# shahcompbio/MultiModalMuSig.jl

Hardware: AMD Instinct MI355X
Metric: E-step docs/sec (higher is better)
Workload: dtype f64; 1 GPU; LDA K=10 alpha=eta=0.1, 10000 docs x 96 SNV terms (BASELINE configs[1]), nnz(rank 0)=913480, one EM iteration per step; docs_rank0=10000, docs_total=10000, terms=96, topics=10, allreduce=none, comm_nranks=1, devices_visible=1

## Files before the change

multimodalmusig.jl_amd/csrc/lda.hip:

```cpp
#include <memory>
#include "dev_math.h"
#include "mmm_logtab.h"
#include "mmm_exptab.h"
#include "mmm_internal.h"

namespace {

constexpr int kWavesPerBlock = 4;
constexpr int kBlock = kWavesPerBlock * MMM_WAVE;
constexpr int kMaxWavesE = 12;

struct LdaDev {
    int D, V, K;
    const int64_t* doc_ptr;
    const int2* tc;
    double alpha, eta;
    const int2* ell;
    const int* dense;
    int Vp;
    const unsigned short* dense16;
};

struct LdaCtl {
    unsigned int ticket;
    int stop;
    int stop_iter;
    int t;
    int n_hist;
    int wait_timeout;
    int pad[2];
};

struct Ring { double* s[3]; };

template <bool RB, class T>
__device__ __forceinline__ T* rep(T* p, size_t n) { return RB ? p + (size_t)blockIdx.y * n : p; }

__device__ __forceinline__ void cell_store(unsigned long long* c, double v, unsigned int seq)
{
    const unsigned long long bits = (unsigned long long)__double_as_longlong(v), tag = (unsigned long long)seq << 32;
    __hip_atomic_store(c, (bits & 0xffffffffull) | tag, __ATOMIC_RELAXED, __HIP_MEMORY_SCOPE_AGENT);
    __hip_atomic_store(c + 1, (bits >> 32) | tag, __ATOMIC_RELAXED, __HIP_MEMORY_SCOPE_AGENT);
// ... 25 lines not shown
#pragma unroll
        for (int j = 0; j < MAXJ; ++j) {
            if (pending & (1u << j)) {
                w0[j] = __hip_atomic_load(c + 2 * (lane + 64 * j), __ATOMIC_RELAXED, __HIP_MEMORY_SCOPE_AGENT);
                w1[j] = __hip_atomic_load(c + 2 * (lane + 64 * j) + 1, __ATOMIC_RELAXED, __HIP_MEMORY_SCOPE_AGENT);
            }
        }
#pragma unroll
        for (int j = 0; j < MAXJ; ++j) {
            if ((pending & (1u << j)) && (unsigned int)(w0[j] >> 32) == seq && (unsigned int)(w1[j] >> 32) == seq) {
                val[j] = __longlong_as_double((long long)((w0[j] & 0xffffffffull) | (w1[j] << 32)));
                pending &= ~(1u << j);
            }
        }
        if (pending) __builtin_amdgcn_s_sleep(1);
    }
    if (pending) ctl->wait_timeout = 1;
    double v = 0.0;
#pragma unroll
    for (int j = 0; j < MAXJ; ++j) v += val[j];
    return v;
}

constexpr int kIldaMaxI = 8, kIldaMaxSJ = 512;

struct EstepArgs {
    LdaDev c;
    const LdaCtl* ctl;
    Ring gamma, Elntheta, expElnbeta, beta;
    double* partial;
    double* llpart;
    int do_ll;
    int t;
    int pstride;
    const double* aexp;
};

#ifdef MMM_DIAG_STAMPS
__device__ unsigned long long g_lda_stamps[16];
#define MMM_STAMP(i)                                                                                         \
    do {                                                                                                     \
        unsigned long long t_;                                                                               \
        __builtin_amdgcn_sched_barrier(0);                                                                   \
        asm volatile("s_memtime %0\n\ts_waitcnt lgkmcnt(0)" : "=s"(t_)::"memory");                          \
        __builtin_amdgcn_sched_barrier(0);                                                                   \
        if (blockIdx.x == 0 && threadIdx.x == 0) g_lda_stamps[i] = t_;                                       \
        if ((i) == 0 || (i) == 7) {                                                                          \
            unsigned long long r_ = __builtin_amdgcn_s_memrealtime();                                        \
            if (blockIdx.x == 0 && threadIdx.x == 0) g_lda_stamps[8 + ((i) != 0)] = r_;                     \
            if (blockIdx.x == gridDim.x - 1 && threadIdx.x == 0) g_lda_stamps[10 + ((i) != 0)] = r_;        \
        }                                                                                                    \
    } while (0)
__device__ unsigned long long g_red_stamps[32];
__device__ unsigned long long g_ll_times[2][512];
#define MMM_LLSTAMP(which, lb)                                                                               \
    do {                                                                                                     \
        __builtin_amdgcn_sched_barrier(0);                                                                   \
        unsigned long long r_ = __builtin_amdgcn_s_memrealtime();                                            \
// ... 57 lines not shown
    bool theta_valid = false;
    bool attr_e[2] = {false, false}, attr_m = false, attr_mm[3] = {false, false, false};
    int cap_mm[3] = {-1, -1, -1}, cap_m = -1;
    DevBuf<unsigned long long> cells;
    DevBuf<unsigned long long> fcells;
    unsigned int kseq = 0;
    bool stop_seen = false;
    bool lag_ll = true;
    bool phi_table_beta = false;
    bool single_step = false;
    bool wide = false;
    DevBuf<int64_t> term_ptr;
    DevBuf<int2> tpost;
    DevBuf<double> aexp;
    DevBuf<double> aexp_next;
    int aexp_for = -1;
    bool pro_used = false;
    DevBuf<double> tabT;
    int stats_waves = 1;
    bool attr_big = false, attr_bigs = false;
    int grid_e = 1, waves_e = 8, grid_s = 1;
    size_t lds_e = 0, lds_tab = 0;
    bool block_stats = false;
    size_t lds_b = 0; bool attr_b = false;
    bool ilda = false;
    IldaDesc ids{};
    DevBuf<int> features;
    DevBuf<double> ilam[3], iEln[3], ibeta[3];
    int R = 1, sel = 0;
    std::vector<int> rep_t, rep_hist;
    PinnedCtl pin;
    LdaDev dev() const { return LdaDev{D, V, K, doc_ptr.p, tc.p, alpha, eta, tc_ell.p, (drows && !cnt16.p) ? cnt_dense.p : nullptr, 16 * SLs, cnt16.p}; }
    int cur() const { return t % 3; }
    Ring ring(DevBuf<double>* b) const { return Ring{{b[0].p, b[1].p, b[2].p}}; }
    double* tab(DevBuf<double>* b, int s) const { return b[s].p + (size_t)sel * V * K; }
    double* doc(DevBuf<double>* b, int s) const { return b[s].p + (size_t)sel * K * D; }
    LdaCtl* ctlp() const { return ctl.p + sel; }
    double* hist() const { return ll_hist.p + (size_t)sel * cap_hist; }
    size_t lds_red() const { return sizeof(double) * ((size_t)KP * V + 64 * (size_t)KP + MMM_LOGTAB_N); }
    int docs_per_ll_block() const { return 16 * (MMM_WAVE / (KP <= 15 ? 16 : (KP <= 31 ? 32 : 64))); }
    void passes_enqueued(bool lag, bool table_beta)
    {
        inflight = true; lag_ll = lag; phi_table_beta = table_beta;
        if (!lag) ll_pending = false;
        phi_valid = false; phi_from_prev = true; gnext_valid = true; theta_valid = false;
    }
};

namespace {

int pick_kp(int K)
{
    static const int opts[] = {2, 4, 6, 8, 10, 12, 16, 20, 24, 32};
    for (int o : opts) if (K <= o) return o;
    if (K <= 64 * kLdaSlots) return (K + 1) & ~1;
// ... 27 lines not shown
{
    mmm_ctx* ctx = m->ctx;
    int nb = 0;
    MMM_HIP(ctx, hipOccupancyMaxActiveBlocksPerMultiprocessor(&nb, (const void*)kern, 1024, lds));
    *cap = nb * std::max(1, ctx->num_cu - 4);
    if (m->tune.resident_cap > 0) *cap = std::min(*cap, m->tune.resident_cap);
    return MMM_OK;
}

template <int KPV, int LV, bool LLV, int VT, bool SG, bool RB>
int go_estep3(mmm_lda* m, const EstepArgs& a)
{
    mmm_ctx* ctx = m->ctx;
    auto k = k_lda_estep<KPV, LV, LLV, VT, SG, RB>;
    if (!m->attr_e[LLV]) { int rc = set_lds(ctx, k, m->lds_e); if (rc) return rc; m->attr_e[LLV] = true; }
    hipLaunchKernelGGL(k, dim3(m->grid_e, RB ? m->R : 1), dim3(m->waves_e * MMM_WAVE), m->lds_e, ctx->stream, a);
    return MMM_OK;
}

template <int KPV, int VT, bool RB>
int go_estep_block(mmm_lda* m, const EstepArgs& a)
{
    mmm_ctx* ctx = m->ctx;
    auto k = k_lda_estep_block<KPV, VT, RB>;
    if (!m->attr_b) { int rc = set_lds(ctx, k, m->lds_b); if (rc) return rc; m->attr_b = true; }
    hipLaunchKernelGGL(k, dim3(m->grid_e, RB ? m->R : 1), dim3(m->waves_e * MMM_WAVE), m->lds_b, ctx->stream, a);
    return MMM_OK;
}

template <int KPV, int LV, bool LLV, int VT, bool RB>
int go_estep2(mmm_lda* m, const EstepArgs& a)
{
    if constexpr (LV == 16 && KPV <= 12 && !LLV) { if (m->single_step && m->block_stats) return go_estep_block<KPV, VT, RB>(m, a); }
    if constexpr (LV == 16 && KPV <= 12) { if (m->single_step) return go_estep3<KPV, LV, LLV, VT, true, RB>(m, a); }
    return go_estep3<KPV, LV, LLV, VT, false, RB>(m, a);
}

template <int KPV, int LV, bool LLV, bool RB = false>
int go_estep(mmm_lda* m, const EstepArgs& a)
{
    if constexpr (LV == 16 && (KPV == 8 || KPV == 10)) { if (m->V == 96) return go_estep2<KPV, LV, LLV, 96, RB>(m, a); }
    return go_estep2<KPV, LV, LLV, 0, RB>(m, a);
}

template <int KPV, int SLV, bool RB = false>
int go_dense(mmm_lda* m, const EstepArgs& a)
{
    if constexpr (KPV * SLV <= 64) {
        mmm_ctx* ctx = m->ctx;
        const bool c16 = m->cnt16.p != nullptr;
        auto k = c16 ? k_lda_estep_dense<KPV, SLV, true, RB> : k_lda_estep_dense<KPV, SLV, false, RB>;
        if (!m->attr_d) { int rc = set_lds(ctx, k, m->lds_d); if (rc) return rc; m->attr_d = true; }
        hipLaunchKernelGGL(k, dim3(m->grid_e, RB ? m->R : 1), dim3(m->waves_e * MMM_WAVE), m->lds_d, ctx->stream, a, (const int*)m->cnt_dense.p, (const unsigned short*)m->cnt16.p);
        return MMM_OK;
    } else return mmm_fail(m->ctx, MMM_ERR_UNSUPPORTED, "LDA: no dense-row build for KP=%d SL=%d", KPV, SLV);
}

int dense_slots(int V) { return V <= 32 ? 2 : (V <= 48 ? 3 : (V <= 96 ? 6 : (V <= 128 ? 8 : 0))); }

template <bool RB = false>
int launch_estep(mmm_lda* m, const EstepArgs& a)
{
    mmm_ctx* ctx = m->ctx;
    int rc = MMM_OK;
    if (m->dense && !a.do_ll) {
        MMM_KP_SWITCH(m, {
            if constexpr (KPV >= 4 && KPV <= 16) {
                switch (m->SL) {
                    case 2: rc = go_dense<KPV, 2, RB>(m, a); break;
                    case 3: rc = go_dense<KPV, 3, RB>(m, a); break;
                    case 6: rc = go_dense<KPV, 6, RB>(m, a); break;
                    default: rc = go_dense<KPV, 8, RB>(m, a); break;
                }
            }
        })
        if (rc) return rc;
        MMM_LAUNCH_CHECK(ctx);
        return MMM_OK;
    }
    if constexpr (RB) {
        if (m->wide || a.do_ll) return mmm_fail(ctx, MMM_ERR_UNSUPPORTED, "LDA batch: no batched build of the wide path / the E-step ll");
        MMM_KP_SWITCH(m, {
            if (m->L == 16) { if constexpr (KPV <= 16) rc = go_estep<KPV, 16, false, true>(m, a); }
            else if (m->L == 32) { if constexpr (KPV >= 16) rc = go_estep<KPV, 32, false, true>(m, a); }
            else { if constexpr (KPV == 32) rc = go_estep<KPV, 64, false, true>(m, a); }
        })
        if (rc) return rc;
// ... 1242 lines not shown
```

multimodalmusig.jl_amd/csrc/lda_estep.cuh:

```cuda
__device__ __forceinline__ void lds_wave_sync()
{
    __builtin_amdgcn_fence(__ATOMIC_SEQ_CST, "wavefront");
    __builtin_amdgcn_wave_barrier();
}

template <bool RB = false>
struct EstepPass {
    const double* __restrict__ gam; const double* __restrict__ gprev; double* __restrict__ gnext; double* __restrict__ Eln;
    const double* __restrict__ eB; const double* __restrict__ bprev;
    __device__ __forceinline__ explicit EstepPass(const EstepArgs& a)
        : gam(a.gamma.s[a.t % 3]), gprev(a.gamma.s[(a.t + 2) % 3]), gnext(a.gamma.s[(a.t + 1) % 3]), Eln(a.Elntheta.s[a.t % 3]),
          eB(a.expElnbeta.s[(a.t + 2) % 3]), bprev(a.beta.s[(a.t + 2) % 3])
    {
        if constexpr (RB) {
            const size_t KD = (size_t)a.c.K * a.c.D, VK = (size_t)a.c.V * a.c.K;
            gam = rep<RB>(gam, KD); gprev = rep<RB>(gprev, KD); gnext = rep<RB>(gnext, KD); Eln = rep<RB>(Eln, KD);
            eB = rep<RB>(eB, VK); bprev = rep<RB>(bprev, VK);
        }
    }
    static __device__ __forceinline__ int stop(const EstepArgs& a) { return rep<RB>(a.ctl, 1)->stop; }
    static __device__ __forceinline__ double* partial(const EstepArgs& a, const int K)
    {
        double* out = a.partial + (size_t)blockIdx.x * K * a.pstride;
        if constexpr (RB) out += (size_t)blockIdx.y * gridDim.x * K * a.pstride;
        return out;
    }
};

template <int KP, bool LL>
__device__ __forceinline__ void lda_chunk(const int2 tcv, const bool act, const int V, const double (&av)[KP], double (&acc)[KP],
                                          const double* __restrict__ sB, const double* __restrict__ sBeta,
                                          const double* __restrict__ myT, double* __restrict__ slab, double& ll_acc)
{
    const double n = (double)tcv.y;
    if (LL) {
        const double* bc = sBeta + tcv.x;
        double p0 = 0.0, p1 = 0.0;
#pragma unroll
        for (int k = 0; k + 1 < KP; k += 2) { p0 = fma(myT[k], bc[k * V], p0); p1 = fma(myT[k + 1], bc[(k + 1) * V], p1); }
        if (KP & 1) p0 = fma(myT[KP - 1], bc[(KP - 1) * V], p0);
        ll_acc = fma(n, dev_log_pos(p0 + p1), ll_acc);
        __builtin_amdgcn_sched_barrier(0);
    }
// ... 16 lines not shown
    double b[KP], s0 = 0.0, s1 = 0.0;
#pragma unroll
    for (int k = 0; k < KP; ++k) b[k] = av[k] * bcol[k * V];
#pragma unroll
    for (int k = 0; k + 1 < KP; k += 2) { s0 += b[k]; s1 += b[k + 1]; }
    if (KP & 1) s0 += b[KP - 1];
    const double r = act ? n * dev_rcp(s0 + s1) : 0.0;
#pragma unroll
    for (int k = 0; k < KP; ++k) { b[k] *= r; acc[k] += b[k]; }
    if (act) {
        double* scol = slab + tcv.x;
#pragma unroll
        for (int k = 0; k < KP; ++k) unsafeAtomicAdd(&scol[k * V], b[k]);
    }
}

template <int KP, int L, bool LL, int VT, bool SINGLE, bool RB = false>
__global__ __launch_bounds__(SINGLE ? kMaxWavesE * MMM_WAVE : 512, SINGLE ? 3 : 2) void k_lda_estep(EstepArgs a)
{
    extern __shared__ __attribute__((aligned(16))) double smem[];
    constexpr int G = MMM_WAVE / L;
    constexpr int PRE = (96 + L - 1) / L;
    MMM_STAMP(0);
    const int stop = EstepPass<RB>::stop(a);
    const EstepPass<RB> io(a);
    const int K = a.c.K, D = a.c.D;
    const int V = VT ? VT : a.c.V;
    const int NW = blockDim.x >> 6;
    const int tid = threadIdx.x, lane = tid & 63, wid = tid >> 6;
    const int g = lane / L, l = lane % L;
    double* sB = smem;
    double* sBeta = sB + (size_t)KP * V;
    double* sSlab = sBeta + (size_t)KP * V;
    double* sA = sSlab + (size_t)NW * KP * V;
    double* sT = sA + (size_t)NW * G * KP;
    double* slab = sSlab + (size_t)wid * KP * V;
    double* myA = sA + ((size_t)wid * G + g) * KP;
    double* myT = sT + ((size_t)wid * G + g) * KP;
    const int stride = gridDim.x * NW * G;
    int base = (blockIdx.x * NW + wid) * G;
    double ll_acc = 0.0;

    int d = base + g;
    bool valid = d < D;
    const bool ext = SINGLE && !LL && !RB && a.aexp != nullptr;
    double gk = ext ? ((valid && l < K) ? a.aexp[(size_t)d * K + l] : 0.0) : ((valid && l < K) ? io.gam[(size_t)d * K + l] : (l < K ? 1.0 : 0.0));
    double gp = (LL && valid && l < K) ? io.gprev[(size_t)d * K + l] : (l < K ? 1.0 : 0.0);
// ... 13 lines not shown
        if (LL) sBeta[i] = (i < K * V) ? io.bprev[i] : 0.0;
    }
    MMM_STAMP(1);

    int d1 = 0; bool valid1 = false; int64_t start1 = 0; int W1 = 0;
    if (!SINGLE) {
        d1 = base + stride + g; valid1 = (base + stride < D) && d1 < D;
        start1 = (valid1 && !rows) ? a.c.doc_ptr[d1] : 0;
        W1 = (valid1 && !rows) ? (int)(a.c.doc_ptr[d1 + 1] - start1) : 0;
    }
    int2 tcp[PRE];
    bool first = true;
    for (;;) {
        const int NCHR = VT ? (VT + L - 1) / L : (V + L - 1) / L;
        const int nch = rows ? NCHR : (W + L - 1) / L;
        const int rot = nch > 0 ? g % nch : 0;
        const int2* __restrict__ tcd = a.c.tc + start;
        int nchmax = nch;
        if (!rows) {
            if (G >= 2) nchmax = max(nchmax, __shfl_xor(nchmax, 32, MMM_WAVE));
            if (G >= 4) nchmax = max(nchmax, __shfl_xor(nchmax, 16, MMM_WAVE));
            nchmax = __builtin_amdgcn_readfirstlane(nchmax);
        }
        if (SINGLE || first) lda_row_read<L, PRE, true, true, true>(a.c, drows, rows, d, valid, l, V, nch, rot, start, W, [&](int j, int w, int n) { tcp[j] = make_int2(w, n); });
        double el = 0.0;
        if (ext) { if (l < KP) myA[l] = gk; }
        else {
            el = lda_elntheta<L>(gk, g, l, K);
            if (l < KP) myA[l] = (l < K) ? ar_exp(el) : 0.0;
        }
        if (LL) {
            const double Sp = group_sum<L>(gp);
            if (l < KP) myT[l] = (l < K) ? gp / Sp : 0.0;
        }
        if (first) {
            if (stop) return;
            if (SINGLE) {
#pragma unroll
                for (int q = 0; q < TB; ++q) { const int i = tid + q * (int)blockDim.x; if (i < KP * V) sB[i] = tb[q]; }
                for (int i = tid + TB * (int)blockDim.x; i < KP * V; i += blockDim.x) sB[i] = (i < K * V) ? io.eB[i] : 0.0;
            }
            __syncthreads();
            first = false;
            MMM_STAMP(2);
        } else lds_wave_sync();
        if (!ext && valid && l < K) io.Eln[(size_t)d * K + l] = el;
        MMM_STAMP(3);
        int2 tcn[PRE];
        double gkn = 0.0, gpn = 0.0;
        int d2 = 0; bool valid2 = false; int64_t start2 = 0; int W2 = 0;
        const bool more = !SINGLE && base + stride < D;
        if (more) {
            const int nch1 = rows ? NCHR : (W1 + L - 1) / L;
            const int rot1 = nch1 > 0 ? g % nch1 : 0;
            lda_row_read<L, PRE, true, true, true>(a.c, drows, rows, d1, valid1, l, V, nch1, rot1, start1, W1, [&](int j, int w, int n) { tcn[j] = make_int2(w, n); });
            gkn = (valid1 && l < K) ? io.gam[(size_t)d1 * K + l] : (l < K ? 1.0 : 0.0);
            gpn = (LL && valid1 && l < K) ? io.gprev[(size_t)d1 * K + l] : (l < K ? 1.0 : 0.0);
            d2 = base + 2 * stride + g; valid2 = (base + 2 * stride < D) && d2 < D;
            start2 = (valid2 && !rows) ? a.c.doc_ptr[d2] : 0;
            W2 = (valid2 && !rows) ? (int)(a.c.doc_ptr[d2 + 1] - start2) : 0;
        }
        {
            double av[KP], acc[KP];
#pragma unroll
            for (int k = 0; k < KP; ++k) { av[k] = myA[k]; acc[k] = 0.0; }
            if (rows) {
#pragma unroll
                for (int j = 0; j < PRE; ++j) {
                    if (j < NCHR) {
                        int2 tcv = tcp[j];
                        const bool act = tcv.x >= 0;
                        tcv.x = act ? tcv.x : 0;
                        lda_chunk<KP, LL>(tcv, act, V, av, acc, sB, sBeta, myT, slab, ll_acc);
                    }
                }
            } else
#pragma unroll 2
            for (int j = 0; j < nchmax; ++j) {
// ... 49 lines not shown
        }
    }
    MMM_STAMP(7);
}


template <int KP>
__device__ __forceinline__ double lda_chunk_r(const int v, const double n, const bool act, const int V, const double (&av)[KP], double (&acc)[KP],
                                              const double* __restrict__ sB)
{
    const double* bcol = sB + v;
    double b[KP], s0 = 0.0, s1 = 0.0;
#pragma unroll
    for (int k = 0; k < KP; ++k) b[k] = bcol[k * V];
#pragma unroll
    for (int k = 0; k + 1 < KP; k += 2) { s0 = fma(av[k], b[k], s0); s1 = fma(av[k + 1], b[k + 1], s1); }
    if (KP & 1) s0 = fma(av[KP - 1], b[KP - 1], s0);
    const double r = act ? n * dev_rcp(s0 + s1) : 0.0;
#pragma unroll
    for (int k = 0; k < KP; ++k) acc[k] = fma(b[k], r, acc[k]);
    return r;
}

template <int KP, int VT, bool RB = false>
__global__ __launch_bounds__(kMaxWavesE * MMM_WAVE, 3) void k_lda_estep_block(EstepArgs a)
{
    static_assert(KP <= 12 && KP % 2 == 0, "topic pairs, table of <= 5 registers per thread");
    extern __shared__ __attribute__((aligned(16))) double smem[];
    constexpr int L = 16, G = MMM_WAVE / L, PRE = 96 / L;
    MMM_STAMP(0);
    const int stop = EstepPass<RB>::stop(a);
    const EstepPass<RB> io(a);
    const int K = a.c.K, D = a.c.D;
    const int V = VT ? VT : a.c.V;
    const int NCHR = VT ? (VT + L - 1) / L : (V + L - 1) / L;
    const int Vs = NCHR * L;
    const int NW = blockDim.x >> 6, ND = NW * G;
    const int tid = threadIdx.x, lane = tid & 63, wid = tid >> 6;
    const int g = lane / L, l = lane % L;
    double* sB = smem;
    double* sR = sB + (size_t)KP * V;
    double* sA = sR + (size_t)ND * Vs;
    double* myR = sR + (size_t)(wid * G + g) * Vs;
    double* myA = sA + (size_t)(wid * G + g) * KP;

    const int d = (blockIdx.x * NW + wid) * G + g;
    const bool valid = d < D;
    const bool ext = !RB && a.aexp != nullptr;
    const double gk = ext ? ((valid && l < K) ? a.aexp[(size_t)d * K + l] : 0.0) : ((valid && l < K) ? io.gam[(size_t)d * K + l] : (l < K ? 1.0 : 0.0));
    const bool drows = a.c.dense != nullptr || a.c.dense16 != nullptr;
    const bool rows = drows || a.c.ell != nullptr;
    const int64_t start = (valid && !rows) ? a.c.doc_ptr[d] : 0;
    const int W = (valid && !rows) ? (int)(a.c.doc_ptr[d + 1] - start) : 0;
    constexpr int TB = KP <= 10 ? 4 : 5;
    double tb[TB];
#pragma unroll
    for (int q = 0; q < TB; ++q) { const int i = tid + q * (int)blockDim.x; tb[q] = (i < K * V) ? io.eB[i] : 0.0; }
    if (!drows) for (int i = tid; i < ND * Vs; i += blockDim.x) sR[i] = 0.0;
    MMM_STAMP(1);

    int tv[PRE]; double tn[PRE];
    const int nch = rows ? NCHR : (W + L - 1) / L;
    lda_row_read<L, PRE, false, true, true>(a.c, drows, rows, d, valid, l, V, nch, 0, start, W, [&](int j, int w, int n) { tv[j] = w; tn[j] = (double)n; });
    double el = 0.0, al = gk;
    if (!ext) {
        el = lda_elntheta<L>(gk, g, l, K);
        al = (l < K) ? ar_exp(el) : 0.0;
    }
    if (l < KP) myA[l] = al;
    if (stop) return;
#pragma unroll
    for (int q = 0; q < TB; ++q) { const int i = tid + q * (int)blockDim.x; if (i < KP * V) sB[i] = tb[q]; }
    for (int i = tid + TB * (int)blockDim.x; i < KP * V; i += blockDim.x) sB[i] = (i < K * V) ? io.eB[i] : 0.0;
    __syncthreads();
    MMM_STAMP(2);
    if (!ext && valid && l < K) io.Eln[(size_t)d * K + l] = el;
    MMM_STAMP(3);
    double av[KP], acc[KP];
#pragma unroll
    for (int k = 0; k < KP; ++k) { av[k] = myA[k]; acc[k] = 0.0; }
    int nchmax = nch;
    if (!rows) {
        nchmax = max(nchmax, __shfl_xor(nchmax, 32, MMM_WAVE));
        nchmax = max(nchmax, __shfl_xor(nchmax, 16, MMM_WAVE));
        nchmax = __builtin_amdgcn_readfirstlane(nchmax);
    }
#pragma unroll
    for (int j = 0; j < PRE; ++j) {
        if (j < nchmax) {
            const bool act = tv[j] >= 0;
            const double r = lda_chunk_r<KP>(act ? tv[j] : 0, tn[j], act, V, av, acc, sB);
            if (drows) myR[j * L + l] = r;
            else if (act) myR[tv[j]] = r;
        }
    }
// ... 194 lines not shown
```

multimodalmusig.jl_amd/csrc/lda_reduce.cuh:

```cuda
struct ReduceArgs {
    const double* partial; const double* llpart; int nslab; int VK;
    double* stats;
    LdaCtl* ctl;
    int t;
    int hist_stride;
    double Nglobal, tol;
    double* ll_hist;
    int do_ll, conv_base, run_tail;
    int p2p; unsigned int p2p_seq; P2PArgs px;
    const double* llpart2; int n_ll, ll_in_k2;
    unsigned long long* ll_cells; unsigned int ll_seq;
};

template <bool RB>
__device__ __forceinline__ void rep_reduce(ReduceArgs& r)
{
    if constexpr (RB) {
        const size_t y = blockIdx.y;
        r.partial += y * r.nslab * r.VK; r.llpart += y * r.nslab; r.stats += y * (r.VK + 16);
        r.ctl += y; r.ll_hist += y * r.hist_stride; r.llpart2 += y * 512;
    }
}

__device__ void lda_pass_tail(const ReduceArgs& r)
// ... 12 lines not shown
    if (!stop) r.ctl->t = r.t;
    r.ctl->ticket = 0;
}

template <bool P2P>
__device__ __forceinline__ void lda_tail_block(const ReduceArgs& r, int lane)
{
    double v = 0.0;
    const bool from_parts = r.ll_in_k2 && !r.ll_cells;
    if (from_parts && r.do_ll) {
        for (int i = lane; i < r.n_ll; i += 64) v += r.llpart2[i];
        v = wave_sum(v);
    }
    if (lane != 0) return;
    if (from_parts) {
        if (r.do_ll) {
            if (P2P && r.p2p) { p2p_send(r.px, r.p2p_seq, r.VK, v); v = p2p_recv_sum(r.px, r.p2p_seq, r.VK, v); }
            r.stats[r.VK] = v;
        }
    } else if (P2P && r.p2p) r.stats[r.VK] = p2p_recv_sum(r.px, r.p2p_seq, r.VK, r.stats[r.VK]);
    lda_pass_tail(r);
}

template <int KP, int L>
__device__ void lda_ll_block(const LdaDev& c, const double* __restrict__ gprev, const double* __restrict__ bprev, double* llpart2, int lb, int nlb,
                             double* smem, unsigned long long* cell = nullptr, unsigned int seq = 0)
{
    __shared__ double s_w[16];
    const int tid = threadIdx.y * 16 + threadIdx.x, lane = tid & 63, wid = tid >> 6;
    constexpr int G = MMM_WAVE / L;
    const int g = lane / L, l = lane % L;
    const int K = c.K, V = c.V, D = c.D;
    double* sBeta = smem;
    double* myT = smem + (size_t)KP * V + ((size_t)wid * G + g) * KP;
    double* sLog = smem + (size_t)KP * V + (size_t)64 * KP;
    const int wslot = ((int64_t)nlb * 16 * G >= (int64_t)D) ? wid * nlb + lb : lb * 16 + wid, nslots = nlb * 16;
    int base = wslot * G;
    int d = base + g;
    bool valid = d < D;
    double gp = (valid && l < K) ? gprev[(size_t)d * K + l] : (l < K ? 1.0 : 0.0);
    constexpr int PRE = 128 / L;
    const bool dense = L == 16 && (c.dense != nullptr || c.dense16 != nullptr);
    const bool h16 = c.dense16 != nullptr;
    const bool ell = dense || c.ell != nullptr;
    int2 pre[PRE];
    const bool fast = L == 16 && dense && h16 && (int64_t)D * K * 8 < ((int64_t)1 << 32) && (int64_t)D * c.Vp * 2 < ((int64_t)1 << 32);
    unsigned wq[4] = {0u, 0u, 0u, 0u};
    const int lk = l < K ? l : K - 1;
    unsigned dl = valid ? (unsigned)d : 0u;
    if (fast) {
        const unsigned* row = at_byte((const unsigned*)c.dense16, (dl * 16u + (unsigned)l) * (unsigned)(c.Vp >> 4) * 2u);
#pragma unroll
        for (int j = 0; j < 4; ++j) wq[j] = row[j];
    } else if (ell) lda_row_read<L, PRE, false, false, false>(c, dense, ell, d, valid, l, V, 0, 0, 0, 0, [&](int j, int w, int n) { pre[j] = make_int2(w, n); });
    int64_t start = (!ell && valid) ? c.doc_ptr[d] : 0;
    int W = (!ell && valid) ? (int)(c.doc_ptr[d + 1] - start) : 0;
    for (int i = tid; i < KP * V; i += 1024) { const int v = i / KP, k = i - v * KP; sBeta[i] = (k < K) ? bprev[(size_t)k * V + v] : 0.0; }
    if (tid < MMM_LOGTAB_N) sLog[tid] = g_mmm_logtab[tid];
    MMM_RSTAMP(lb == 0 && tid == 0, 20);
    __syncthreads();
    MMM_RSTAMP(lb == 0 && tid == 0, 21);
    double acc = 0.0;
    if (fast) {
        const int nch = (V + L - 1) / L;
        const int stride = nslots * G;
        const unsigned slp2 = (unsigned)(c.Vp >> 4) * 2u;
        unsigned w[4];
#pragma unroll
        for (int j = 0; j < 4; ++j) w[j] = valid ? wq[j] : 0u;
        for (; base < D; base += stride) {
            const int dn = d + stride;
            const bool validn = base + stride < D && dn < D;
            const unsigned dnl = validn ? (unsigned)dn : dl;
            const double Sp = group_sum<L>(gp);
            lds_wave_sync();
            if (l < KP) myT[l] = (l < K) ? dev_div(gp, Sp) : 0.0;
            lds_wave_sync();
            double tv[KP];
#pragma unroll
            for (int k = 0; k < KP; ++k) tv[k] = myT[k];
            double gpn = *at_byte(gprev, (dnl * (unsigned)K + (unsigned)lk) * 8u);
            {
                const unsigned* row = at_byte((const unsigned*)c.dense16, (dnl * 16u + (unsigned)l) * slp2);
// ... 3 lines not shown
#pragma unroll
            for (int j = 0; j < 8; ++j) {
                if (j < nch) {
                    const unsigned cq = (j & 1) ? w[j / 2] >> 16 : w[j / 2] & 0xffffu;
                    const bool act = valid && j * L + l < V;
                    acc = lda_ll_term<KP>(tv, sBeta + (size_t)(act ? j * L + l : 0) * KP, act, (double)cq, sLog, acc);
                }
            }
            asm volatile("" : "+v"(acc) :: "memory");
            asm volatile("" : "+v"(gpn) :: "memory");
#pragma unroll
            for (int j = 0; j < 4; ++j) asm volatile("" : "+v"(wq[j]) :: "memory");
            d = dn; valid = validn; dl = dnl;
            gp = (valid && l < K) ? gpn : (l < K ? 1.0 : 0.0);
#pragma unroll
            for (int j = 0; j < 4; ++j) w[j] = valid ? wq[j] : 0u;
        }
    } else if (ell) {
        const int nch = (V + L - 1) / L;
        for (; base < D; base += nslots * G) {
            if (base != wslot * G) {
                d = base + g; valid = d < D;
                gp = (valid && l < K) ? gprev[(size_t)d * K + l] : (l < K ? 1.0 : 0.0);
                lda_row_read<L, PRE, false, false, false>(c, dense, ell, d, valid, l, V, 0, 0, 0, 0, [&](int j, int w, int n) { pre[j] = make_int2(w, n); });
            }
            const double Sp = group_sum<L>(gp);
            lds_wave_sync();
            if (l < KP) myT[l] = (l < K) ? dev_div(gp, Sp) : 0.0;
            lds_wave_sync();
            double tv[KP];
#pragma unroll
            for (int k = 0; k < KP; ++k) tv[k] = myT[k];
#pragma unroll
            for (int j = 0; j < PRE; ++j) {
                if (j >= nch) break;
                const int2 t = pre[j];
                const bool act = t.x >= 0;
                acc = lda_ll_term<KP>(tv, sBeta + (size_t)(act ? t.x : 0) * KP, act, (double)t.y, sLog, acc);
            }
        }
    } else
    for (; base < D; base += nslots * G) {
        if (base != wslot * G) {
            d = base + g; valid = d < D;
            gp = (valid && l < K) ? gprev[(size_t)d * K + l] : (l < K ? 1.0 : 0.0);
            start = valid ? c.doc_ptr[d] : 0;
            W = valid ? (int)(c.doc_ptr[d + 1] - start) : 0;
// ... 8 lines not shown
        for (int k = 0; k < KP; ++k) tv[k] = myT[k];
        int nchmax = (W + L - 1) / L;
        if (G >= 2) nchmax = max(nchmax, __shfl_xor(nchmax, 32, MMM_WAVE));
        if (G >= 4) nchmax = max(nchmax, __shfl_xor(nchmax, 16, MMM_WAVE));
        nchmax = __builtin_amdgcn_readfirstlane(nchmax);
        for (int j = 0; j < nchmax; ++j) {
            const int w = j * L + l;
            const bool act = w < W;
            const int2 t = act ? tcd[w] : make_int2(0, 0);
            acc = lda_ll_term<KP>(tv, sBeta + (size_t)t.x * KP, act, (double)t.y, sLog, acc);
        }
    }
    MMM_RSTAMP(lb == 0 && tid == 0, 22);
    acc = wave_sum(acc);
    if (lane == 0) s_w[wid] = acc;
    __syncthreads();
    MMM_RSTAMP(lb == 0 && tid == 0, 23);
    if (tid == 0) {
        double v = 0.0;
#pragma unroll
        for (int w = 0; w < 16; ++w) v += s_w[w];
        if (cell) cell_store(cell, v, seq); else llpart2[lb] = v;
    }
}

__device__ void lda_reduce_block(const ReduceArgs& r)
{
    __shared__ double sm[64][17];
    const int stop = r.ctl->stop;
    const int tx = threadIdx.x, ty = threadIdx.y;
    const int e = blockIdx.x * 16 + tx;
    double acc = 0.0;
    if (e < r.VK) for (int sl = ty; sl < r.nslab; sl += 64) acc += r.partial[(size_t)sl * r.VK + e];
    if (stop) {
        if (r.p2p && blockIdx.x == 0 && tx == 0 && ty == 0) p2p_send(r.px, r.p2p_seq, 0, 0.0);
        return;
    }
    sm[ty][tx] = acc;
    __syncthreads();
    if (ty < 8) {
        double v = 0.0;
#pragma unroll
        for (int j = 0; j < 8; ++j) v += sm[ty * 8 + j][tx];
        sm[ty * 8][tx] = v;
    }
    __syncthreads();
    if (ty == 0 && e < r.VK) {
        double v = 0.0;
#pragma unroll
        for (int j = 0; j < 8; ++j) v += sm[j * 8][tx];
        r.stats[e] = v;
        if (r.p2p) p2p_send(r.px, r.p2p_seq, e, v);
    }
    if (blockIdx.x == 0 && ty >= 4 && ty < 8 && r.ll_cells && r.do_ll) {
        const int lane = (ty * 16 + tx) & 63;
        double v = 0.0;
        v = cells_wait_sum(r.ll_cells, r.n_ll, lane, r.ll_seq, r.ctl);
// ... 41 lines not shown
    IldaDesc ds;
    double* ilam; double* iEln; double* ibeta;
    unsigned long long* fcells;
};

struct MergeArgs {
    int V; double eta;
    Ring lambda, Elnbeta, expElnbeta, beta;
    unsigned long long* cells;
    unsigned int seq;
    int nred;
    int ll_join;
    int n_ll;
    int epb, nredp;
    int pro;
    const double* pro_gamma; double* pro_Eln; double* pro_a;
};

template <int KP, bool P2P, bool ILDA>
__global__ __launch_bounds__(1024) void k_lda_reduce_ll_mstep(ReduceArgs r, LdaDev c, const double* gprev, const double* bprev, MergeArgs ms, IldaMerge im)
{
    extern __shared__ __attribute__((aligned(16))) double smem[];
    __shared__ double sm2[2][64][17];
    const int stop = r.ctl->stop;
    const int tx = threadIdx.x, ty = threadIdx.y, tid = ty * 16 + tx;
    MMM_RSTAMP(blockIdx.x == 1 && tid == 0, 0);
    MMM_RSTAMP(blockIdx.x == 0 && tid == 64, 8);
    MMM_RSTAMP((int)blockIdx.x == ms.nredp && tid == 0, 16);
    if ((int)blockIdx.x >= ms.nredp) {
        if (stop) return;
        constexpr int L = KP <= 15 ? 16 : (KP <= 31 ? 32 : 64);
        const int lb = (int)blockIdx.x - ms.nredp, n_ll = ms.n_ll;
        MMM_LLSTAMP(0, lb);
        double gnx = 0.0;
        int pd = 0;
        if constexpr (KP <= 12) {
            if (ms.pro) {
                const int lane = tid & 63, l = lane & 15;
                pd = ((tid >> 6) * n_ll + lb) * 4 + (lane >> 4);
                gnx = (pd < c.D && l < c.K) ? ms.pro_gamma[(size_t)pd * c.K + l] : (l < c.K ? 1.0 : 0.0);
            }
        }
        lda_ll_block<KP, L>(c, gprev, bprev, nullptr, lb, n_ll + (ms.ll_join ? ms.nredp - 1 : 0), smem, ms.cells + 2 * (ms.nred + lb), ms.seq);
        MMM_RSTAMP((int)blockIdx.x == ms.nredp && tid == 0, 17);
        MMM_LLSTAMP(1, lb);
        if constexpr (KP <= 12) {
            if (ms.pro) {
                const int lane = tid & 63, g = lane >> 4, l = lane & 15, K = c.K;
                const double el = lda_elntheta<16>(gnx, g, l, K);
                if (pd < c.D && l < K) { ms.pro_Eln[(size_t)pd * K + l] = el; ms.pro_a[(size_t)pd * K + l] = ar_exp(el); }
            }
        }
        return;
    }
    const int rbp = (int)blockIdx.x, epb = ms.epb;
    const int rb = rbp * epb + (ty < epb ? ty : 0);
    const int e = rb * 16 + tx;
    double acc = 0.0, acc1 = 0.0;
    {
        const int e0 = rbp * epb * 16 + tx;
        if (epb == 2) {
            for (int sl = ty; sl < r.nslab; sl += 64) { acc += r.partial[(size_t)sl * r.VK + e0]; acc1 += r.partial[(size_t)sl * r.VK + e0 + 16]; }
        } else {
            for (int sl = ty; sl < r.nslab; sl += 64) acc += r.partial[(size_t)sl * r.VK + e0];
        }
    }
    if (stop) {
        if (P2P && rbp == 0 && tid == 0) { p2p_send(r.px, r.p2p_seq, 0, 0.0); (void)p2p_recv_sum(r.px, r.p2p_seq, 0, 0.0); }
        return;
    }
    MMM_RSTAMP(blockIdx.x == 1 && tid == 0, 1);
    sm2[0][ty][tx] = acc; sm2[1][ty][tx] = acc1;
    __syncthreads();
    if (ty < 8) {
#pragma unroll
        for (int h = 0; h < 2; ++h) {
            double v = 0.0;
#pragma unroll
            for (int j = 0; j < 8; ++j) v += sm2[h][ty * 8 + j][tx];
            sm2[h][ty * 8][tx] = v;
        }
    }
    __syncthreads();
    double (*sm)[17] = sm2[ty < epb ? ty : 0];
    MMM_RSTAMP(blockIdx.x == 1 && tid == 0, 2);
    if (ty < epb) {
        double v = 0.0;
#pragma unroll
        for (int j = 0; j < 8; ++j) v += sm[j * 8][tx];
        if (P2P) { p2p_send(r.px, r.p2p_seq, e, v); v = p2p_recv_sum(r.px, r.p2p_seq, e, v); }
// ... 257 lines not shown
```

multimodalmusig.jl_amd/csrc/lda_rows.cuh:

```cuda

__device__ __forceinline__ int row_slot(int w, int slp) { return (w & 15) * slp + (w >> 4); }
__device__ __forceinline__ int row16_count(unsigned w0, unsigned w1, unsigned w2, unsigned w3, int c)
{
    const unsigned word = c < 4 ? (c < 2 ? w0 : w1) : (c < 6 ? w2 : w3);
    return (int)((c & 1) ? word >> 16 : word & 0xffffu);
}

template <int L, int PRE, bool ROT, bool ZERO_OFF, bool WIDE16, class Put>
__device__ __forceinline__ void lda_row_read(const LdaDev& c, const bool counts, const bool pairs, const int d, const bool valid, const int l, const int V,
                                             const int nch, const int rot, const int64_t start, const int W, Put&& put)
{
    auto chunk = [&](int j) { int q = j; if (ROT) { q += rot; if (q >= nch) q -= nch; } return q; };
    if (counts) {
        const int* __restrict__ row = c.dense + (size_t)(valid ? d : 0) * c.Vp;
        const unsigned short* __restrict__ row16 = c.dense16 + (size_t)(valid ? d : 0) * c.Vp;
        const bool h16 = c.dense16 != nullptr;
        const int slp = c.Vp >> 4;
        if (WIDE16 && L == 16 && h16) {
            const unsigned* __restrict__ r32 = (const unsigned*)(row16 + (size_t)l * slp);
            const unsigned w0 = r32[0], w1 = r32[1], w2 = r32[2], w3 = r32[3];
#pragma unroll
            for (int j = 0; j < PRE; ++j) {
                const int q = chunk(j), w = q * L + l;
                const bool in = valid && (!ROT || j < nch) && w < V;
                const int n = in ? row16_count(w0, w1, w2, w3, q) : 0;
                put(j, (ZERO_OFF ? n > 0 : in) ? w : -1, n);
            }
        } else
#pragma unroll
        for (int j = 0; j < PRE; ++j) {
            const int q = chunk(j), w = q * L + l;
            const bool in = valid && (!ROT || j < nch) && w < V;
            const int n = in ? (h16 ? (int)row16[row_slot(w, slp)] : row[row_slot(w, slp)]) : 0;
            put(j, (ZERO_OFF ? n > 0 : in) ? w : -1, n);
        }
    } else {
        const int2* __restrict__ src = pairs ? c.ell + (size_t)(valid ? d : 0) * V : c.tc + start;
        const int lim = pairs ? (valid ? V : 0) : W;
#pragma unroll
        for (int j = 0; j < PRE; ++j) {
            const int w = chunk(j) * L + l;
            const int2 p = ((!ROT || j < nch) && w < lim) ? src[w] : make_int2(-1, 0);
            put(j, p.x, p.y);
        }
    }
}

template <int L>
__device__ __forceinline__ double lda_elntheta(const double gk, const int g, const int l, const int K)
{
    const double S = group_sum<L>(gk);
    const double ps = dev_digamma_pos(l < K ? gk : S);
    return ps - __shfl(ps, g * L + K, MMM_WAVE);
}

template <int KP>
__device__ __forceinline__ double lda_ll_term(const double (&tv)[KP], const double* bc, const bool act, const double count, const double* sLog, const double acc)
{
    double p0 = 0.0, p1 = 0.0;
#pragma unroll
    for (int k = 0; k + 1 < KP; k += 2) { p0 = fma(tv[k], bc[k], p0); p1 = fma(tv[k + 1], bc[k + 1], p1); }
    if (KP & 1) p0 = fma(tv[KP - 1], bc[KP - 1], p0);
    const double p = act ? p0 + p1 : 1.0;
    return fma(count, dev_log_tab(p, sLog), acc);
}
```

Measured before the change: 629.0 million docs/s.

## Hoist loads ahead of stop checks, resolve ring slots on host, group row loads

```diff
diff --git a/multimodalmusig.jl_amd/csrc/lda.hip b/multimodalmusig.jl_amd/csrc/lda.hip
--- a/multimodalmusig.jl_amd/csrc/lda.hip
+++ b/multimodalmusig.jl_amd/csrc/lda.hip
@@ -12,12 +12,12 @@
 
 struct LdaDev {
     int D, V, K;
+    int Vp;
     const int64_t* doc_ptr;
     const int2* tc;
     double alpha, eta;
     const int2* ell;
     const int* dense;
-    int Vp;
     const unsigned short* dense16;
 };
 
@@ -89,6 +89,9 @@
     return v;
 }
 
+__device__ __forceinline__ int lda_stop_request(const LdaCtl* ctl) { return __hip_atomic_load(&ctl->stop, __ATOMIC_RELAXED, __HIP_MEMORY_SCOPE_AGENT); }
+__device__ __forceinline__ bool lda_stop_now(int requested) { return __builtin_amdgcn_readfirstlane(requested) != 0; }
+
 constexpr int kIldaMaxI = 8, kIldaMaxSJ = 512;
 
 struct EstepArgs {
@@ -101,6 +104,11 @@
     int t;
     int pstride;
     const double* aexp;
+    struct Slots { const double* gam; const double* gprev; double* gnext; double* Eln; const double* eB; const double* bprev; } now;
+    void resolve()
+    {
+        now = Slots{gamma.s[t % 3], gamma.s[(t + 2) % 3], gamma.s[(t + 1) % 3], Elntheta.s[t % 3], expElnbeta.s[(t + 2) % 3], beta.s[(t + 2) % 3]};
+    }
 };
 
 #ifdef MMM_DIAG_STAMPS
@@ -204,7 +212,7 @@
     int grid_e = 1, waves_e = 8, grid_s = 1;
     size_t lds_e = 0, lds_tab = 0;
     bool block_stats = false;
-    size_t lds_b = 0; bool attr_b = false;
+    size_t lds_b = 0; bool attr_b[2] = {false, false};
     bool ilda = false;
     IldaDesc ids{};
     DevBuf<int> features;
@@ -212,7 +220,7 @@
     int R = 1, sel = 0;
     std::vector<int> rep_t, rep_hist;
     PinnedCtl pin;
-    LdaDev dev() const { return LdaDev{D, V, K, doc_ptr.p, tc.p, alpha, eta, tc_ell.p, (drows && !cnt16.p) ? cnt_dense.p : nullptr, 16 * SLs, cnt16.p}; }
+    LdaDev dev() const { return LdaDev{D, V, K, 16 * SLs, doc_ptr.p, tc.p, alpha, eta, tc_ell.p, (drows && !cnt16.p) ? cnt_dense.p : nullptr, cnt16.p}; }
     int cur() const { return t % 3; }
     Ring ring(DevBuf<double>* b) const { return Ring{{b[0].p, b[1].p, b[2].p}}; }
     double* tab(DevBuf<double>* b, int s) const { return b[s].p + (size_t)sel * V * K; }
@@ -286,8 +294,9 @@
 int go_estep_block(mmm_lda* m, const EstepArgs& a)
 {
     mmm_ctx* ctx = m->ctx;
-    auto k = k_lda_estep_block<KPV, VT, RB>;
-    if (!m->attr_b) { int rc = set_lds(ctx, k, m->lds_b); if (rc) return rc; m->attr_b = true; }
+    const bool r16 = !RB && a.c.dense16 != nullptr;
+    auto k = r16 ? k_lda_estep_block<KPV, VT, RB, !RB> : k_lda_estep_block<KPV, VT, RB, false>;
+    if (!m->attr_b[r16]) { int rc = set_lds(ctx, k, m->lds_b); if (rc) return rc; m->attr_b[r16] = true; }
     hipLaunchKernelGGL(k, dim3(m->grid_e, RB ? m->R : 1), dim3(m->waves_e * MMM_WAVE), m->lds_b, ctx->stream, a);
     return MMM_OK;
 }
@@ -323,10 +332,12 @@
 int dense_slots(int V) { return V <= 32 ? 2 : (V <= 48 ? 3 : (V <= 96 ? 6 : (V <= 128 ? 8 : 0))); }
 
 template <bool RB = false>
-int launch_estep(mmm_lda* m, const EstepArgs& a)
+int launch_estep(mmm_lda* m, const EstepArgs& pass)
 {
     mmm_ctx* ctx = m->ctx;
     int rc = MMM_OK;
+    EstepArgs a = pass;
+    a.resolve();
     if (m->dense && !a.do_ll) {
         MMM_KP_SWITCH(m, {
             if constexpr (KPV >= 4 && KPV <= 16) {
diff --git a/multimodalmusig.jl_amd/csrc/lda_estep.cuh b/multimodalmusig.jl_amd/csrc/lda_estep.cuh
--- a/multimodalmusig.jl_amd/csrc/lda_estep.cuh
+++ b/multimodalmusig.jl_amd/csrc/lda_estep.cuh
@@ -9,8 +9,7 @@
     const double* __restrict__ gam; const double* __restrict__ gprev; double* __restrict__ gnext; double* __restrict__ Eln;
     const double* __restrict__ eB; const double* __restrict__ bprev;
     __device__ __forceinline__ explicit EstepPass(const EstepArgs& a)
-        : gam(a.gamma.s[a.t % 3]), gprev(a.gamma.s[(a.t + 2) % 3]), gnext(a.gamma.s[(a.t + 1) % 3]), Eln(a.Elntheta.s[a.t % 3]),
-          eB(a.expElnbeta.s[(a.t + 2) % 3]), bprev(a.beta.s[(a.t + 2) % 3])
+        : gam(a.now.gam), gprev(a.now.gprev), gnext(a.now.gnext), Eln(a.now.Eln), eB(a.now.eB), bprev(a.now.bprev)
     {
         if constexpr (RB) {
             const size_t KD = (size_t)a.c.K * a.c.D, VK = (size_t)a.c.V * a.c.K;
@@ -18,7 +17,7 @@
             eB = rep<RB>(eB, VK); bprev = rep<RB>(bprev, VK);
         }
     }
-    static __device__ __forceinline__ int stop(const EstepArgs& a) { return rep<RB>(a.ctl, 1)->stop; }
+    static __device__ __forceinline__ int stop_request(const EstepArgs& a) { return lda_stop_request(rep<RB>(a.ctl, 1)); }
     static __device__ __forceinline__ double* partial(const EstepArgs& a, const int K)
     {
         double* out = a.partial + (size_t)blockIdx.x * K * a.pstride;
@@ -81,7 +80,7 @@
     constexpr int G = MMM_WAVE / L;
     constexpr int PRE = (96 + L - 1) / L;
     MMM_STAMP(0);
-    const int stop = EstepPass<RB>::stop(a);
+    const int stop = EstepPass<RB>::stop_request(a);
     const EstepPass<RB> io(a);
     const int K = a.c.K, D = a.c.D;
     const int V = VT ? VT : a.c.V;
@@ -141,7 +140,7 @@
             if (G >= 4) nchmax = max(nchmax, __shfl_xor(nchmax, 16, MMM_WAVE));
             nchmax = __builtin_amdgcn_readfirstlane(nchmax);
         }
-        if (SINGLE || first) lda_row_read<L, PRE, true, true, true>(a.c, drows, rows, d, valid, l, V, nch, rot, start, W, [&](int j, int w, int n) { tcp[j] = make_int2(w, n); });
+        if (SINGLE || first) lda_row_read<L, PRE, true, true, true, true>(a.c, drows, rows, d, valid, l, V, nch, rot, start, W, [&](int j, int w, int n) { tcp[j] = make_int2(w, n); });
         double el = 0.0;
         if (ext) { if (l < KP) myA[l] = gk; }
         else {
@@ -153,7 +152,7 @@
             if (l < KP) myT[l] = (l < K) ? gp / Sp : 0.0;
         }
         if (first) {
-            if (stop) return;
+            if (lda_stop_now(stop)) return;
             if (SINGLE) {
 #pragma unroll
                 for (int q = 0; q < TB; ++q) { const int i = tid + q * (int)blockDim.x; if (i < KP * V) sB[i] = tb[q]; }
@@ -172,7 +171,7 @@
         if (more) {
             const int nch1 = rows ? NCHR : (W1 + L - 1) / L;
             const int rot1 = nch1 > 0 ? g % nch1 : 0;
-            lda_row_read<L, PRE, true, true, true>(a.c, drows, rows, d1, valid1, l, V, nch1, rot1, start1, W1, [&](int j, int w, int n) { tcn[j] = make_int2(w, n); });
+            lda_row_read<L, PRE, true, true, true, true>(a.c, drows, rows, d1, valid1, l, V, nch1, rot1, start1, W1, [&](int j, int w, int n) { tcn[j] = make_int2(w, n); });
             gkn = (valid1 && l < K) ? io.gam[(size_t)d1 * K + l] : (l < K ? 1.0 : 0.0);
             gpn = (LL && valid1 && l < K) ? io.gprev[(size_t)d1 * K + l] : (l < K ? 1.0 : 0.0);
             d2 = base + 2 * stride + g; valid2 = (base + 2 * stride < D) && d2 < D;
@@ -268,14 +267,16 @@
     return r;
 }
 
-template <int KP, int VT, bool RB = false>
+template <int KP, int VT, bool RB = false, bool R16 = false>
 __global__ __launch_bounds__(kMaxWavesE * MMM_WAVE, 3) void k_lda_estep_block(EstepArgs a)
 {
     static_assert(KP <= 12 && KP % 2 == 0, "topic pairs, table of <= 5 registers per thread");
     extern __shared__ __attribute__((aligned(16))) double smem[];
     constexpr int L = 16, G = MMM_WAVE / L, PRE = 96 / L;
     MMM_STAMP(0);
-    const int stop = EstepPass<RB>::stop(a);
+    asm volatile("" :: "s"(a.ctl), "s"(a.aexp), "s"(a.now.gam), "s"(a.now.gnext), "s"(a.now.Eln), "s"(a.now.eB), "s"(a.c.dense16), "s"(a.c.dense), "s"(a.c.ell),
+                 "s"(a.c.doc_ptr), "s"(a.c.tc), "s"(a.c.Vp), "s"(a.c.D), "s"(a.c.K), "s"(a.c.V), "s"(a.c.alpha), "s"(a.partial), "s"(a.pstride), "s"((int)blockDim.x));
+    const int stop = EstepPass<RB>::stop_request(a);
     const EstepPass<RB> io(a);
     const int K = a.c.K, D = a.c.D;
     const int V = VT ? VT : a.c.V;
@@ -292,31 +293,41 @@
 
     const int d = (blockIdx.x * NW + wid) * G + g;
     const bool valid = d < D;
+    const int dl = valid ? d : 0;
     const bool ext = !RB && a.aexp != nullptr;
-    const double gk = ext ? ((valid && l < K) ? a.aexp[(size_t)d * K + l] : 0.0) : ((valid && l < K) ? io.gam[(size_t)d * K + l] : (l < K ? 1.0 : 0.0));
-    const bool drows = a.c.dense != nullptr || a.c.dense16 != nullptr;
+    const double* __restrict__ gsrc = ext ? a.aexp : io.gam;
+    const double graw = gsrc[(size_t)dl * K + (l < K ? l : K - 1)];
+    const bool drows = R16 || a.c.dense != nullptr || a.c.dense16 != nullptr;
     const bool rows = drows || a.c.ell != nullptr;
-    const int64_t start = (valid && !rows) ? a.c.doc_ptr[d] : 0;
-    const int W = (valid && !rows) ? (int)(a.c.doc_ptr[d + 1] - start) : 0;
     constexpr int TB = KP <= 10 ? 4 : 5;
     double tb[TB];
 #pragma unroll
-    for (int q = 0; q < TB; ++q) { const int i = tid + q * (int)blockDim.x; tb[q] = (i < K * V) ? io.eB[i] : 0.0; }
+    for (int q = 0; q < TB; ++q) { const int i = tid + q * (int)blockDim.x; tb[q] = io.eB[i < K * V ? i : K * V - 1]; }
+    int64_t start = 0; int W = 0;
+    if constexpr (!R16) {
+        start = (valid && !rows) ? a.c.doc_ptr[d] : 0;
+        W = (valid && !rows) ? (int)(a.c.doc_ptr[d + 1] - start) : 0;
+    }
+    unsigned w16[4] = {0u, 0u, 0u, 0u};
+    if constexpr (R16) lda_row16_load(a.c, dl, l, w16);
     if (!drows) for (int i = tid; i < ND * Vs; i += blockDim.x) sR[i] = 0.0;
     MMM_STAMP(1);
 
     int tv[PRE]; double tn[PRE];
     const int nch = rows ? NCHR : (W + L - 1) / L;
-    lda_row_read<L, PRE, false, true, true>(a.c, drows, rows, d, valid, l, V, nch, 0, start, W, [&](int j, int w, int n) { tv[j] = w; tn[j] = (double)n; });
+    auto put = [&](int j, int w, int n) { tv[j] = w; tn[j] = (double)n; };
+    if constexpr (R16) lda_row16_put<L, PRE, false, true>(w16, valid, l, V, nch, 0, put);
+    else lda_row_read<L, PRE, false, true, true, true>(a.c, drows, rows, d, valid, l, V, nch, 0, start, W, put);
+    const double gk = (valid && l < K) ? graw : ((ext || l >= K) ? 0.0 : 1.0);
     double el = 0.0, al = gk;
     if (!ext) {
         el = lda_elntheta<L>(gk, g, l, K);
         al = (l < K) ? ar_exp(el) : 0.0;
     }
     if (l < KP) myA[l] = al;
-    if (stop) return;
-#pragma unroll
-    for (int q = 0; q < TB; ++q) { const int i = tid + q * (int)blockDim.x; if (i < KP * V) sB[i] = tb[q]; }
+    if (lda_stop_now(stop)) return;
+#pragma unroll
+    for (int q = 0; q < TB; ++q) { const int i = tid + q * (int)blockDim.x; if (i < KP * V) sB[i] = (i < K * V) ? tb[q] : 0.0; }
     for (int i = tid + TB * (int)blockDim.x; i < KP * V; i += blockDim.x) sB[i] = (i < K * V) ? io.eB[i] : 0.0;
     __syncthreads();
     MMM_STAMP(2);
diff --git a/multimodalmusig.jl_amd/csrc/lda_reduce.cuh b/multimodalmusig.jl_amd/csrc/lda_reduce.cuh
--- a/multimodalmusig.jl_amd/csrc/lda_reduce.cuh
+++ b/multimodalmusig.jl_amd/csrc/lda_reduce.cuh
@@ -58,9 +58,9 @@
     lda_pass_tail(r);
 }
 
-template <int KP, int L>
-__device__ void lda_ll_block(const LdaDev& c, const double* __restrict__ gprev, const double* __restrict__ bprev, double* llpart2, int lb, int nlb,
-                             double* smem, unsigned long long* cell = nullptr, unsigned int seq = 0)
+template <int KP, int L, bool EARLY = false>
+__device__ bool lda_ll_block(const LdaDev& c, const double* __restrict__ gprev, const double* __restrict__ bprev, double* llpart2, int lb, int nlb,
+                             double* smem, unsigned long long* cell = nullptr, unsigned int seq = 0, const int stop = 0)
 {
     __shared__ double s_w[16];
     const int tid = threadIdx.y * 16 + threadIdx.x, lane = tid & 63, wid = tid >> 6;
@@ -88,13 +88,24 @@
         const unsigned* row = at_byte((const unsigned*)c.dense16, (dl * 16u + (unsigned)l) * (unsigned)(c.Vp >> 4) * 2u);
 #pragma unroll
         for (int j = 0; j < 4; ++j) wq[j] = row[j];
-    } else if (ell) lda_row_read<L, PRE, false, false, false>(c, dense, ell, d, valid, l, V, 0, 0, 0, 0, [&](int j, int w, int n) { pre[j] = make_int2(w, n); });
+    } else if (ell) lda_row_read<L, PRE, false, false, false, false>(c, dense, ell, d, valid, l, V, 0, 0, 0, 0, [&](int j, int w, int n) { pre[j] = make_int2(w, n); });
     int64_t start = (!ell && valid) ? c.doc_ptr[d] : 0;
     int W = (!ell && valid) ? (int)(c.doc_ptr[d + 1] - start) : 0;
-    for (int i = tid; i < KP * V; i += 1024) { const int v = i / KP, k = i - v * KP; sBeta[i] = (k < K) ? bprev[(size_t)k * V + v] : 0.0; }
-    if (tid < MMM_LOGTAB_N) sLog[tid] = g_mmm_logtab[tid];
+    if constexpr (EARLY) {
+        const double lt = g_mmm_logtab[tid & (MMM_LOGTAB_N - 1)];
+        for (int i = tid; i < KP * V; i += 1024) {
+            const int v = i / KP, k = i - v * KP;
+            const double b = bprev[(size_t)(k < K ? k : K - 1) * V + v];
+            sBeta[i] = (k < K) ? b : 0.0;
+        }
+        if (tid < MMM_LOGTAB_N) sLog[tid] = lt;
+    } else {
+        for (int i = tid; i < KP * V; i += 1024) { const int v = i / KP, k = i - v * KP; sBeta[i] = (k < K) ? bprev[(size_t)k * V + v] : 0.0; }
+        if (tid < MMM_LOGTAB_N) sLog[tid] = g_mmm_logtab[tid];
+    }
     MMM_RSTAMP(lb == 0 && tid == 0, 20);
     __syncthreads();
+    if constexpr (EARLY) { if (lda_stop_now(stop)) return true; }
     MMM_RSTAMP(lb == 0 && tid == 0, 21);
     double acc = 0.0;
     if (fast) {
@@ -144,7 +155,7 @@
             if (base != wslot * G) {
                 d = base + g; valid = d < D;
                 gp = (valid && l < K) ? gprev[(size_t)d * K + l] : (l < K ? 1.0 : 0.0);
-                lda_row_read<L, PRE, false, false, false>(c, dense, ell, d, valid, l, V, 0, 0, 0, 0, [&](int j, int w, int n) { pre[j] = make_int2(w, n); });
+                lda_row_read<L, PRE, false, false, false, false>(c, dense, ell, d, valid, l, V, 0, 0, 0, 0, [&](int j, int w, int n) { pre[j] = make_int2(w, n); });
             }
             const double Sp = group_sum<L>(gp);
             lds_wave_sync();
@@ -199,17 +210,18 @@
         for (int w = 0; w < 16; ++w) v += s_w[w];
         if (cell) cell_store(cell, v, seq); else llpart2[lb] = v;
     }
+    return false;
 }
 
 __device__ void lda_reduce_block(const ReduceArgs& r)
 {
     __shared__ double sm[64][17];
-    const int stop = r.ctl->stop;
+    const int stop_req = lda_stop_request(r.ctl);
     const int tx = threadIdx.x, ty = threadIdx.y;
     const int e = blockIdx.x * 16 + tx;
     double acc = 0.0;
     if (e < r.VK) for (int sl = ty; sl < r.nslab; sl += 64) acc += r.partial[(size_t)sl * r.VK + e];
-    if (stop) {
+    if (lda_stop_now(stop_req)) {
         if (r.p2p && blockIdx.x == 0 && tx == 0 && ty == 0) p2p_send(r.px, r.p2p_seq, 0, 0.0);
         return;
     }
@@ -297,13 +309,15 @@
 {
     extern __shared__ __attribute__((aligned(16))) double smem[];
     __shared__ double sm2[2][64][17];
-    const int stop = r.ctl->stop;
+    asm volatile("" :: "s"(r.ctl), "s"(r.partial), "s"(r.nslab), "s"(r.VK), "s"(c.D), "s"(c.V), "s"(c.K), "s"(c.Vp), "s"(c.doc_ptr), "s"(c.tc), "s"(c.ell),
+                 "s"(c.dense), "s"(c.dense16), "s"(gprev), "s"(bprev), "s"(ms.nredp), "s"(ms.nred), "s"(ms.n_ll), "s"(ms.ll_join), "s"(ms.epb), "s"(ms.pro),
+                 "s"(ms.pro_gamma), "s"(ms.cells), "s"(ms.seq));
+    const int stop_req = lda_stop_request(r.ctl);
     const int tx = threadIdx.x, ty = threadIdx.y, tid = ty * 16 + tx;
     MMM_RSTAMP(blockIdx.x == 1 && tid == 0, 0);
     MMM_RSTAMP(blockIdx.x == 0 && tid == 64, 8);
     MMM_RSTAMP((int)blockIdx.x == ms.nredp && tid == 0, 16);
     if ((int)blockIdx.x >= ms.nredp) {
-        if (stop) return;
         constexpr int L = KP <= 15 ? 16 : (KP <= 31 ? 32 : 64);
         const int lb = (int)blockIdx.x - ms.nredp, n_ll = ms.n_ll;
         MMM_LLSTAMP(0, lb);
@@ -313,16 +327,16 @@
             if (ms.pro) {
                 const int lane = tid & 63, l = lane & 15;
                 pd = ((tid >> 6) * n_ll + lb) * 4 + (lane >> 4);
-                gnx = (pd < c.D && l < c.K) ? ms.pro_gamma[(size_t)pd * c.K + l] : (l < c.K ? 1.0 : 0.0);
-            }
-        }
-        lda_ll_block<KP, L>(c, gprev, bprev, nullptr, lb, n_ll + (ms.ll_join ? ms.nredp - 1 : 0), smem, ms.cells + 2 * (ms.nred + lb), ms.seq);
+                gnx = ms.pro_gamma[(size_t)(pd < c.D ? pd : 0) * c.K + (l < c.K ? l : c.K - 1)];
+            }
+        }
+        if (lda_ll_block<KP, L, true>(c, gprev, bprev, nullptr, lb, n_ll + (ms.ll_join ? ms.nredp - 1 : 0), smem, ms.cells + 2 * (ms.nred + lb), ms.seq, stop_req)) return;
         MMM_RSTAMP((int)blockIdx.x == ms.nredp && tid == 0, 17);
         MMM_LLSTAMP(1, lb);
         if constexpr (KP <= 12) {
             if (ms.pro) {
                 const int lane = tid & 63, g = lane >> 4, l = lane & 15, K = c.K;
-                const double el = lda_elntheta<16>(gnx, g, l, K);
+                const double el = lda_elntheta<16>((pd < c.D && l < K) ? gnx : (l < K ? 1.0 : 0.0), g, l, K);
                 if (pd < c.D && l < K) { ms.pro_Eln[(size_t)pd * K + l] = el; ms.pro_a[(size_t)pd * K + l] = ar_exp(el); }
             }
         }
@@ -340,7 +354,7 @@
             for (int sl = ty; sl < r.nslab; sl += 64) acc += r.partial[(size_t)sl * r.VK + e0];
         }
     }
-    if (stop) {
+    if (lda_stop_now(stop_req)) {
         if (P2P && rbp == 0 && tid == 0) { p2p_send(r.px, r.p2p_seq, 0, 0.0); (void)p2p_recv_sum(r.px, r.p2p_seq, 0, 0.0); }
         return;
     }
diff --git a/multimodalmusig.jl_amd/csrc/lda_rows.cuh b/multimodalmusig.jl_amd/csrc/lda_rows.cuh
--- a/multimodalmusig.jl_amd/csrc/lda_rows.cuh
+++ b/multimodalmusig.jl_amd/csrc/lda_rows.cuh
@@ -6,7 +6,26 @@
     return (int)((c & 1) ? word >> 16 : word & 0xffffu);
 }
 
-template <int L, int PRE, bool ROT, bool ZERO_OFF, bool WIDE16, class Put>
+__device__ __forceinline__ void lda_row16_load(const LdaDev& c, const int dl, const int l, unsigned (&w)[4])
+{
+    const unsigned* __restrict__ r32 = (const unsigned*)(c.dense16 + (size_t)dl * c.Vp + (size_t)l * (c.Vp >> 4));
+#pragma unroll
+    for (int q = 0; q < 4; ++q) w[q] = r32[q];
+}
+template <int L, int PRE, bool ROT, bool ZERO_OFF, class Put>
+__device__ __forceinline__ void lda_row16_put(const unsigned (&w4)[4], const bool valid, const int l, const int V, const int nch, const int rot, Put&& put)
+{
+#pragma unroll
+    for (int j = 0; j < PRE; ++j) {
+        int q = j; if (ROT) { q += rot; if (q >= nch) q -= nch; }
+        const int w = q * L + l;
+        const bool in = valid && (!ROT || j < nch) && w < V;
+        const int n = in ? row16_count(w4[0], w4[1], w4[2], w4[3], q) : 0;
+        put(j, (ZERO_OFF ? n > 0 : in) ? w : -1, n);
+    }
+}
+
+template <int L, int PRE, bool ROT, bool ZERO_OFF, bool WIDE16, bool GROUP, class Put>
 __device__ __forceinline__ void lda_row_read(const LdaDev& c, const bool counts, const bool pairs, const int d, const bool valid, const int l, const int V,
                                              const int nch, const int rot, const int64_t start, const int W, Put&& put)
 {
@@ -17,31 +36,60 @@
         const bool h16 = c.dense16 != nullptr;
         const int slp = c.Vp >> 4;
         if (WIDE16 && L == 16 && h16) {
-            const unsigned* __restrict__ r32 = (const unsigned*)(row16 + (size_t)l * slp);
-            const unsigned w0 = r32[0], w1 = r32[1], w2 = r32[2], w3 = r32[3];
+            unsigned w[4];
+            lda_row16_load(c, valid ? d : 0, l, w);
+            lda_row16_put<L, PRE, ROT, ZERO_OFF>(w, valid, l, V, nch, rot, put);
+        } else if constexpr (!GROUP) {
 #pragma unroll
             for (int j = 0; j < PRE; ++j) {
                 const int q = chunk(j), w = q * L + l;
                 const bool in = valid && (!ROT || j < nch) && w < V;
-                const int n = in ? row16_count(w0, w1, w2, w3, q) : 0;
+                const int n = in ? (h16 ? (int)row16[row_slot(w, slp)] : row[row_slot(w, slp)]) : 0;
                 put(j, (ZERO_OFF ? n > 0 : in) ? w : -1, n);
             }
-        } else
+        } else {
+            int n[PRE];
+            if (h16) {
 #pragma unroll
-        for (int j = 0; j < PRE; ++j) {
-            const int q = chunk(j), w = q * L + l;
-            const bool in = valid && (!ROT || j < nch) && w < V;
-            const int n = in ? (h16 ? (int)row16[row_slot(w, slp)] : row[row_slot(w, slp)]) : 0;
-            put(j, (ZERO_OFF ? n > 0 : in) ? w : -1, n);
+                for (int j = 0; j < PRE; ++j) { const int w = chunk(j) * L + l; n[j] = (int)row16[row_slot(w < V ? w : 0, slp)]; }
+            } else {
+#pragma unroll
+                for (int j = 0; j < PRE; ++j) { const int w = chunk(j) * L + l; n[j] = row[row_slot(w < V ? w : 0, slp)]; }
+            }
+            __builtin_amdgcn_sched_barrier(0);
+#pragma unroll
+            for (int j = 0; j < PRE; ++j) {
+                const int w = chunk(j) * L + l;
+                const bool in = valid && (!ROT || j < nch) && w < V;
+                const int nn = in ? n[j] : 0;
+                put(j, (ZERO_OFF ? nn > 0 : in) ? w : -1, nn);
+            }
         }
     } else {
         const int2* __restrict__ src = pairs ? c.ell + (size_t)(valid ? d : 0) * V : c.tc + start;
         const int lim = pairs ? (valid ? V : 0) : W;
+        if constexpr (!GROUP) {
 #pragma unroll
-        for (int j = 0; j < PRE; ++j) {
-            const int w = chunk(j) * L + l;
-            const int2 p = ((!ROT || j < nch) && w < lim) ? src[w] : make_int2(-1, 0);
-            put(j, p.x, p.y);
+            for (int j = 0; j < PRE; ++j) {
+                const int w = chunk(j) * L + l;
+                const int2 p = ((!ROT || j < nch) && w < lim) ? src[w] : make_int2(-1, 0);
+                put(j, p.x, p.y);
+            }
+        } else {
+            int2 p[PRE];
+#pragma unroll
+            for (int j = 0; j < PRE; ++j) {
+                const int w = chunk(j) * L + l;
+                const int2* __restrict__ at = ((!ROT || j < nch) && w < lim) ? src + w : (const int2*)c.doc_ptr;
+                p[j] = *at;
+            }
+            __builtin_amdgcn_sched_barrier(0);
+#pragma unroll
+            for (int j = 0; j < PRE; ++j) {
+                const int w = chunk(j) * L + l;
+                const bool in = (!ROT || j < nch) && w < lim;
+                put(j, in ? p[j].x : -1, in ? p[j].y : 0);
+            }
         }
     }
 }
```

Result: faster. 644.6 million docs/s, median of 6 (+2.5%).
